# akuendig/cuda-matrix-inversion

Hardware: AMD Instinct MI355X
Metric: matrix inversions/s (higher is better)
Workload: dtype f64; 1 GPU; gj64: 100000 x 64x64 fp64 Gauss-Jordan, SPD inputs (natural-order pivots verified inside the MFMA sweep; a rejected matrix is redone with partial pivoting), BASELINE configs[2]; n=64, total_batch=100000, batch_per_gpu=100000, algorithm=gj, kernel=matinv_gj_tile_f64<4, true, true>, input=SPD: R + R^T + n I

## Files before the change

### cuda-matrix-inversion_amd/csrc/tile_gj_kernels.hip

```cpp
#include "tile_impl.hpp"

namespace matinv {

template hipError_t launch_gj_tile<double>(int, BatchRef<const double>, BatchRef<double>, size_t, int *, hipStream_t);

}
```

### cuda-matrix-inversion_amd/csrc/tile_impl.hpp

```cpp
#pragma once
#include <stdio.h>
#include <stdlib.h>
#include <string.h>
#include <atomic>

#include "tile_common.hpp"
#include "tile_screen.hpp"

#ifndef MATINV_TILE_GATED_PANEL
#define MATINV_TILE_GATED_PANEL 1
#endif

#ifndef MATINV_TILE_SYM_SWEEP
#define MATINV_TILE_SYM_SWEEP 1
#endif

namespace matinv {


#define MATINV_PREP_ROW(MOV, b, a) MOV " %" #b ", %" #a "\n\t" MOV " %" #a ", 0\n\t"
#define MATINV_PREP_ZERO(MOV, a) MOV " %" #a ", 0\n\t"
#define MATINV_PREP_TAIL(MOV, save, eye) MOV " %0, %" #eye "\n\ts_nop 1\n\ts_mov_b64 exec, %" #save
#define MATINV_PREP_SAVE(save, mask) "s_and_saveexec_b64 %" #save ", %" #mask "\n\t"
template <int NT, class T>
__device__ __forceinline__ void prep_operands(typename TileGeo<T>::vec4 (&acc)[NT][NT], T (&bop)[NT], int kb, T eye)
{
    static_assert(NT >= 1 && NT <= 4, "prep_operands: one asm text per tile count");
    const int tK = kb >> 2, rK = kb & 3;
    const unsigned long long pmask = sizeof(T) == 8 ? 0x000F000F000F000FULL << (4 * rK) : 0x1111111111111111ULL << rK;
    unsigned long long save;
    auto J = [&](int i) { return (tK + i) % NT; };
    auto R = [&](int i) { return (rK + i) & 3; };
#define ROW(i) acc[tK][J(i)][rK]
#define COL(i, r) acc[J(i)][tK][R(r)]
    if constexpr (sizeof(T) == 8) {
#define MV "v_mov_b64_e32"
        if constexpr (NT == 1)
            asm volatile(MATINV_PREP_ROW(MV, 0, 1) MATINV_PREP_SAVE(5, 6)
                         MATINV_PREP_ZERO(MV, 2) MATINV_PREP_ZERO(MV, 3) MATINV_PREP_ZERO(MV, 4) MATINV_PREP_TAIL(MV, 5, 7)
                         : "=&v"(bop[J(0)]), "+v"(ROW(0)), "+v"(COL(0, 1)), "+v"(COL(0, 2)), "+v"(COL(0, 3)), "=&s"(save)
                         : "s"(pmask), "v"(eye) : "scc");
        else if constexpr (NT == 2)
            asm volatile(MATINV_PREP_ROW(MV, 0, 2) MATINV_PREP_ROW(MV, 1, 3) MATINV_PREP_SAVE(11, 12)
                         MATINV_PREP_ZERO(MV, 4) MATINV_PREP_ZERO(MV, 5) MATINV_PREP_ZERO(MV, 6)
                         MATINV_PREP_ZERO(MV, 7) MATINV_PREP_ZERO(MV, 8) MATINV_PREP_ZERO(MV, 9) MATINV_PREP_ZERO(MV, 10)
                         MATINV_PREP_TAIL(MV, 11, 13)
                         : "=&v"(bop[J(0)]), "=&v"(bop[J(1)]), "+v"(ROW(0)), "+v"(ROW(1)),
                           "+v"(COL(0, 1)), "+v"(COL(0, 2)), "+v"(COL(0, 3)),
                           "+v"(COL(1, 0)), "+v"(COL(1, 1)), "+v"(COL(1, 2)), "+v"(COL(1, 3)), "=&s"(save)
                         : "s"(pmask), "v"(eye) : "scc");
        else if constexpr (NT == 3)
            asm volatile(MATINV_PREP_ROW(MV, 0, 3) MATINV_PREP_ROW(MV, 1, 4) MATINV_PREP_ROW(MV, 2, 5) MATINV_PREP_SAVE(17, 18)
                         MATINV_PREP_ZERO(MV, 6) MATINV_PREP_ZERO(MV, 7) MATINV_PREP_ZERO(MV, 8)
                         MATINV_PREP_ZERO(MV, 9) MATINV_PREP_ZERO(MV, 10) MATINV_PREP_ZERO(MV, 11) MATINV_PREP_ZERO(MV, 12)
                         MATINV_PREP_ZERO(MV, 13) MATINV_PREP_ZERO(MV, 14) MATINV_PREP_ZERO(MV, 15) MATINV_PREP_ZERO(MV, 16)
                         MATINV_PREP_TAIL(MV, 17, 19)
                         : "=&v"(bop[J(0)]), "=&v"(bop[J(1)]), "=&v"(bop[J(2)]), "+v"(ROW(0)), "+v"(ROW(1)), "+v"(ROW(2)),
                           "+v"(COL(0, 1)), "+v"(COL(0, 2)), "+v"(COL(0, 3)),
                           "+v"(COL(1, 0)), "+v"(COL(1, 1)), "+v"(COL(1, 2)), "+v"(COL(1, 3)),
                           "+v"(COL(2, 0)), "+v"(COL(2, 1)), "+v"(COL(2, 2)), "+v"(COL(2, 3)), "=&s"(save)
                         : "s"(pmask), "v"(eye) : "scc");
        else
            asm volatile(MATINV_PREP_ROW(MV, 0, 4) MATINV_PREP_ROW(MV, 1, 5) MATINV_PREP_ROW(MV, 2, 6) MATINV_PREP_ROW(MV, 3, 7)
                         MATINV_PREP_SAVE(23, 24)
                         MATINV_PREP_ZERO(MV, 8) MATINV_PREP_ZERO(MV, 9) MATINV_PREP_ZERO(MV, 10)
                         MATINV_PREP_ZERO(MV, 11) MATINV_PREP_ZERO(MV, 12) MATINV_PREP_ZERO(MV, 13) MATINV_PREP_ZERO(MV, 14)
                         MATINV_PREP_ZERO(MV, 15) MATINV_PREP_ZERO(MV, 16) MATINV_PREP_ZERO(MV, 17) MATINV_PREP_ZERO(MV, 18)
                         MATINV_PREP_ZERO(MV, 19) MATINV_PREP_ZERO(MV, 20) MATINV_PREP_ZERO(MV, 21) MATINV_PREP_ZERO(MV, 22)
                         MATINV_PREP_TAIL(MV, 23, 25)
                         : "=&v"(bop[J(0)]), "=&v"(bop[J(1)]), "=&v"(bop[J(2)]), "=&v"(bop[J(3)]),
                           "+v"(ROW(0)), "+v"(ROW(1)), "+v"(ROW(2)), "+v"(ROW(3)),
                           "+v"(COL(0, 1)), "+v"(COL(0, 2)), "+v"(COL(0, 3)),
                           "+v"(COL(1, 0)), "+v"(COL(1, 1)), "+v"(COL(1, 2)), "+v"(COL(1, 3)),
                           "+v"(COL(2, 0)), "+v"(COL(2, 1)), "+v"(COL(2, 2)), "+v"(COL(2, 3)),
                           "+v"(COL(3, 0)), "+v"(COL(3, 1)), "+v"(COL(3, 2)), "+v"(COL(3, 3)), "=&s"(save)
                         : "s"(pmask), "v"(eye) : "scc");
#undef MV
    } else {
#define MV "v_mov_b32_e32"
        if constexpr (NT == 1)
            asm volatile(MATINV_PREP_ROW(MV, 0, 1) MATINV_PREP_SAVE(5, 6)
                         MATINV_PREP_ZERO(MV, 2) MATINV_PREP_ZERO(MV, 3) MATINV_PREP_ZERO(MV, 4) MATINV_PREP_TAIL(MV, 5, 7)
                         : "=&v"(bop[J(0)]), "+v"(ROW(0)), "+v"(COL(0, 1)), "+v"(COL(0, 2)), "+v"(COL(0, 3)), "=&s"(save)
                         : "s"(pmask), "v"(eye) : "scc");
        else if constexpr (NT == 2)
            asm volatile(MATINV_PREP_ROW(MV, 0, 2) MATINV_PREP_ROW(MV, 1, 3) MATINV_PREP_SAVE(11, 12)
                         MATINV_PREP_ZERO(MV, 4) MATINV_PREP_ZERO(MV, 5) MATINV_PREP_ZERO(MV, 6)
                         MATINV_PREP_ZERO(MV, 7) MATINV_PREP_ZERO(MV, 8) MATINV_PREP_ZERO(MV, 9) MATINV_PREP_ZERO(MV, 10)
                         MATINV_PREP_TAIL(MV, 11, 13)
                         : "=&v"(bop[J(0)]), "=&v"(bop[J(1)]), "+v"(ROW(0)), "+v"(ROW(1)),
                           "+v"(COL(0, 1)), "+v"(COL(0, 2)), "+v"(COL(0, 3)),
                           "+v"(COL(1, 0)), "+v"(COL(1, 1)), "+v"(COL(1, 2)), "+v"(COL(1, 3)), "=&s"(save)
                         : "s"(pmask), "v"(eye) : "scc");
        else if constexpr (NT == 3)
            asm volatile(MATINV_PREP_ROW(MV, 0, 3) MATINV_PREP_ROW(MV, 1, 4) MATINV_PREP_ROW(MV, 2, 5) MATINV_PREP_SAVE(17, 18)
                         MATINV_PREP_ZERO(MV, 6) MATINV_PREP_ZERO(MV, 7) MATINV_PREP_ZERO(MV, 8)
                         MATINV_PREP_ZERO(MV, 9) MATINV_PREP_ZERO(MV, 10) MATINV_PREP_ZERO(MV, 11) MATINV_PREP_ZERO(MV, 12)
                         MATINV_PREP_ZERO(MV, 13) MATINV_PREP_ZERO(MV, 14) MATINV_PREP_ZERO(MV, 15) MATINV_PREP_ZERO(MV, 16)
                         MATINV_PREP_TAIL(MV, 17, 19)
                         : "=&v"(bop[J(0)]), "=&v"(bop[J(1)]), "=&v"(bop[J(2)]), "+v"(ROW(0)), "+v"(ROW(1)), "+v"(ROW(2)),
                           "+v"(COL(0, 1)), "+v"(COL(0, 2)), "+v"(COL(0, 3)),
                           "+v"(COL(1, 0)), "+v"(COL(1, 1)), "+v"(COL(1, 2)), "+v"(COL(1, 3)),
                           "+v"(COL(2, 0)), "+v"(COL(2, 1)), "+v"(COL(2, 2)), "+v"(COL(2, 3)), "=&s"(save)
                         : "s"(pmask), "v"(eye) : "scc");
        else
            asm volatile(MATINV_PREP_ROW(MV, 0, 4) MATINV_PREP_ROW(MV, 1, 5) MATINV_PREP_ROW(MV, 2, 6) MATINV_PREP_ROW(MV, 3, 7)
                         MATINV_PREP_SAVE(23, 24)
                         MATINV_PREP_ZERO(MV, 8) MATINV_PREP_ZERO(MV, 9) MATINV_PREP_ZERO(MV, 10)
                         MATINV_PREP_ZERO(MV, 11) MATINV_PREP_ZERO(MV, 12) MATINV_PREP_ZERO(MV, 13) MATINV_PREP_ZERO(MV, 14)
                         MATINV_PREP_ZERO(MV, 15) MATINV_PREP_ZERO(MV, 16) MATINV_PREP_ZERO(MV, 17) MATINV_PREP_ZERO(MV, 18)
                         MATINV_PREP_ZERO(MV, 19) MATINV_PREP_ZERO(MV, 20) MATINV_PREP_ZERO(MV, 21) MATINV_PREP_ZERO(MV, 22)
                         MATINV_PREP_TAIL(MV, 23, 25)
                         : "=&v"(bop[J(0)]), "=&v"(bop[J(1)]), "=&v"(bop[J(2)]), "=&v"(bop[J(3)]),
                           "+v"(ROW(0)), "+v"(ROW(1)), "+v"(ROW(2)), "+v"(ROW(3)),
                           "+v"(COL(0, 1)), "+v"(COL(0, 2)), "+v"(COL(0, 3)),
                           "+v"(COL(1, 0)), "+v"(COL(1, 1)), "+v"(COL(1, 2)), "+v"(COL(1, 3)),
                           "+v"(COL(2, 0)), "+v"(COL(2, 1)), "+v"(COL(2, 2)), "+v"(COL(2, 3)),
                           "+v"(COL(3, 0)), "+v"(COL(3, 1)), "+v"(COL(3, 2)), "+v"(COL(3, 3)), "=&s"(save)
                         : "s"(pmask), "v"(eye) : "scc");
#undef MV
    }
#undef ROW
#undef COL
}
#undef MATINV_PREP_ROW
#undef MATINV_PREP_ZERO
#undef MATINV_PREP_TAIL
#undef MATINV_PREP_SAVE


__device__ __forceinline__ void note_differs(unsigned long long &asym, double a, double b)
{
    asm volatile("v_cmp_ne_u64_e64 vcc, %1, %2\n\ts_or_b64 %0, %0, vcc" : "+s"(asym) : "v"(a), "v"(b) : "vcc");
}

template <int NT>
__device__ __forceinline__ unsigned long long tile_asymmetry(double *tbuf, const v4d (&acc)[NT][NT], int q, int c)
{
    typedef TileGeo<double> G;
    unsigned long long asym = 0;
#pragma unroll
    for (int ti = 0; ti < NT; ++ti)
#pragma unroll
        for (int tj = 0; tj <= ti; ++tj) {
            if (asym != 0) continue;
            wave_lds_sync();
#pragma unroll
            for (int r = 0; r < 4; ++r) tbuf[G::trow(r, q) * TILE_TSTRIDE + c] = acc[ti][tj][r];
            wave_lds_sync();
#pragma unroll
            for (int r = 0; r < 4; ++r) note_differs(asym, tbuf[c * TILE_TSTRIDE + G::trow(r, q)], acc[tj][ti][r]);
        }
    return asym;
}

__device__ __forceinline__ void pin_tiles(v4d (&acc)[4][4])
{
    asm volatile("" : "+v"(acc[0][0]), "+v"(acc[0][1]), "+v"(acc[0][2]), "+v"(acc[0][3]), "+v"(acc[1][0]), "+v"(acc[1][1]),
                      "+v"(acc[1][2]), "+v"(acc[1][3]), "+v"(acc[2][0]), "+v"(acc[2][1]), "+v"(acc[2][2]), "+v"(acc[2][3]),
                      "+v"(acc[3][0]), "+v"(acc[3][1]), "+v"(acc[3][2]), "+v"(acc[3][3]));
}

template <int NT, bool GATED, class T>
__device__ __forceinline__ void sym_tile_sweep(typename TileGeo<T>::vec4 (&acc)[NT][NT], T *panel, int q, int c, unsigned long long &bad)
{
    typedef TileGeo<T> G;
    typedef PanelSolve<NT, false, T, GATED, true> PS;
    constexpr int NKB = 4 * NT;
    T aop[NT], bop[NT];
    spd_panel_to_lds<NT, T>(panel, acc, 0, q, c);
    wave_lds_sync();
    {
        PS ps0;
#pragma unroll
        for (int s = 0; s < PS::NSTAGE; ++s) ps0.stage(s, panel, 0, q, c, aop, bop, bad);
    }
#pragma unroll
    for (int kb = 0; kb < NKB; ++kb) {
        spd_prep_operands<NT, T>(acc, bop, kb, q, c);
        if (kb + 1 < NKB) {
            const int tn = (kb + 1) >> 2;
#pragma unroll
            for (int ti = tn; ti < NT; ++ti) acc[ti][tn] = G::mfma(aop[ti], bop[tn], acc[ti][tn]);
#pragma unroll
            for (int tj = 0; tj < tn; ++tj) acc[tn][tj] = G::mfma(aop[tn], bop[tj], acc[tn][tj]);
            constexpr int NB = NT * (NT + 1) / 2 - NT;
            constexpr int NS = PS::NSTAGE;
            T aop_next[NT], bop_next[NT];
            PS ps;
            int count = 0, ev = 0;
            auto run_events = [&](bool flush) {
#pragma unroll
                for (int e = 0; e < NS + 1; ++e) {
                    const int lead = NB < 2 ? NB : 2;
                    const int thr = (e == 0) ? lead : lead + ((NB - lead) * e) / NS;
                    if (e == ev && (flush || thr <= count)) {
                        __builtin_amdgcn_sched_barrier(0);
                        if (e == 0) {
                            wave_lds_sync();
                            spd_panel_to_lds<NT, T>(panel, acc, kb + 1, q, c);
                            wave_lds_sync();
                        } else {
                            ps.stage(e - 1, panel, kb + 1, q, c, aop_next, bop_next, bad);
                        }
                        __builtin_amdgcn_sched_barrier(0);
                        ++ev;
                    }
                }
            };
            run_events(false);
#pragma unroll
            for (int ti = 0; ti < NT; ++ti)
#pragma unroll
                for (int tj = 0; tj <= ti; ++tj) {
                    if (ti == tn || tj == tn) continue;
                    acc[ti][tj] = G::mfma(aop[ti], bop[tj], acc[ti][tj]);
                    ++count;
                    run_events(false);
                }
            run_events(true);
#pragma unroll
            for (int ti = 0; ti < NT; ++ti) { aop[ti] = aop_next[ti]; bop[ti] = bop_next[ti]; }
        } else {
#pragma unroll
            for (int ti = 0; ti < NT; ++ti)
#pragma unroll
                for (int tj = 0; tj <= ti; ++tj) acc[ti][tj] = G::mfma(aop[ti], bop[tj], acc[ti][tj]);
        }
    }
}

template <int NT>
__device__ __forceinline__ void sym_tile_finish(double *tbuf, v4d (&acc)[NT][NT], int q, int c)
{
    typedef TileGeo<double> G;
#pragma unroll
    for (int ti = 0; ti < NT; ++ti)
#pragma unroll
        for (int tj = 0; tj <= ti; ++tj) {
            acc[ti][tj] = -acc[ti][tj];
            wave_lds_sync();
#pragma unroll
            for (int r = 0; r < 4; ++r) tbuf[G::trow(r, q) * TILE_TSTRIDE + c] = acc[ti][tj][r];
            wave_lds_sync();
#pragma unroll
            for (int r = 0; r < 4; ++r) {
                const double t = tbuf[c * TILE_TSTRIDE + G::trow(r, q)];
                acc[tj][ti][r] = (ti != tj || G::trow(r, q) < c) ? t : acc[tj][ti][r];
            }
        }
}

template <class T, int NT, bool FULL, bool LOOKAHEAD, bool EARLY = false>
__device__ __forceinline__ void gj_tile_body(BatchRef<const T> Ain, BatchRef<T> Xout, int *info, int n_rt, unsigned batch,
                                             int *work_count, int *work_list, T *panel, const int *in_count, const int *in_list)
{
    typedef TileGeo<T> G;
    typedef typename G::vec4 vec4;
    typedef typename G::vec2 vec2;
    constexpr int N = 16 * NT;
    constexpr int NKB = 4 * NT;
    constexpr bool PAIRED = FULL && (NT % 2 == 0);
    constexpr bool GATED = MATINV_TILE_GATED_PANEL && sizeof(T) == 8 && NT == 4 && FULL && LOOKAHEAD && !EARLY;
    constexpr bool SYM = MATINV_TILE_SYM_SWEEP && sizeof(T) == 8 && NT == 4 && FULL && LOOKAHEAD;
    const int l = threadIdx.x;

    const unsigned todo = in_count ? (unsigned)*in_count : batch;
    for (unsigned item = blockIdx.x; item < todo; item += gridDim.x) {
        const unsigned mat = in_list ? (unsigned)in_list[item] : item;
        const T *A = Ain.at_uniform(mat);
        T *X = Xout.at_uniform(mat);
        int n = FULL ? N : n_rt;
        if (!FULL) asm volatile("" : "+s"(n));
        int q = l >> 4, c = l & 15;
        const unsigned lane_off = (unsigned)(G::trow(0, l >> 4) * n + (l & 15));
        asm volatile("" : "+v"(q), "+v"(c));
        const T eye = G::piv(c) == q ? (T)1 : (T)0;
        vec4 acc[NT][NT];
        if (PAIRED) {
            const unsigned lane_off2 = (unsigned)(2 * G::trow(0, l >> 4) * N + 2 * (l & 15));
#pragma unroll
            for (int ti = 0; ti < NT; ++ti)
#pragma unroll
                for (int u = 0; u < NT / 2; ++u)
#pragma unroll
                    for (int r = 0; r < 4; ++r) {
                        const unsigned uoff = (unsigned)((32 * (ti >> 1) + 2 * G::trow(r, 0) + (ti & 1)) * N + 32 * u);
                        const vec2 v = __builtin_nontemporal_load(reinterpret_cast<const vec2 *>(A + uoff + lane_off2));
                        acc[ti][2 * u][r] = v[0];
                        acc[ti][2 * u + 1][r] = v[1];
                    }
        } else {
#pragma unroll
            for (int ti = 0; ti < NT; ++ti)
#pragma unroll
                for (int tj = 0; tj < NT; ++tj)
#pragma unroll
                    for (int r = 0; r < 4; ++r) {
                        const int row = 16 * ti + G::trow(r, q), col = 16 * tj + c;
                        const unsigned uoff = (unsigned)((16 * ti + G::trow(r, 0)) * n + 16 * tj);
                        const bool edge = !FULL && (ti == NT - 1 || tj == NT - 1);
                        acc[ti][tj][r] = (!edge || (row < n && col < n)) ? A[uoff + lane_off] : ((row == col) ? (T)1 : (T)0);
                    }
        }
        unsigned long long bad = 0;
        T aop[NT], bop[NT];

        bool sym = false;
#ifndef MATINV_TILE_LDST_ONLY
        if constexpr (SYM) {
            pin_tiles(acc);
            sym = tile_asymmetry<NT>(panel, acc, q, c) == 0;
        }
#endif

#ifdef MATINV_TILE_LDST_ONLY
        if (false) {
#else
        if (SYM && sym) {
        } else if (LOOKAHEAD) {
#endif
            panel_to_lds<NT, T>(panel, acc, 0, q, c);
            wave_lds_sync();
            panel_solve<NT, GATED>(panel, 0, q, c, aop, bad);
#pragma unroll
            for (int kb = 0; kb < NKB; ++kb) {
                if (!FULL && kb > 4 * (NT - 1) && kb - 4 * (NT - 1) >= G::real_blocks(n - 16 * (NT - 1))) continue;
                prep_operands<NT, T>(acc, bop, kb, eye);
                if (kb + 1 < NKB) {
                    const int tn = (kb + 1) >> 2;
#pragma unroll
                    for (int ti = 0; ti < NT; ++ti)
                        acc[ti][tn] = G::mfma(aop[ti], bop[tn], acc[ti][tn]);
                    constexpr int NB = NT * (NT - 1);
                    int pend = 0;
                    auto issue_b = [&](int count) {
#pragma unroll
                        for (int z = 0; z < count; ++z) {
                            if (pend < NB) {
                                const int tjx = pend / NT, ti = pend % NT;
                                const int tj = tjx + (tjx >= tn ? 1 : 0);
                                acc[ti][tj] = G::mfma(aop[ti], bop[tj], acc[ti][tj]);
                                ++pend;
                            }
                        }
                        __builtin_amdgcn_sched_barrier(0);
                    };
                    __builtin_amdgcn_sched_barrier(0);
                    issue_b(2);
                    wave_lds_sync();
                    panel_to_lds<NT, T>(panel, acc, kb + 1, q, c);
                    wave_lds_sync();
                    __builtin_amdgcn_sched_barrier(0);
                    T aop_next[NT];
                    PanelSolve<NT, false, T, GATED> ps;
                    constexpr int NS = PanelSolve<NT, false, T, GATED>::NSTAGE;
#pragma unroll
                    for (int s = 0; s < NS; ++s) {
                        issue_b(((NB - 2) * (s + 1)) / NS - ((NB - 2) * s) / NS);
                        ps.stage(s, panel, kb + 1, q, c, aop_next, bad);
                        __builtin_amdgcn_sched_barrier(0);
                    }
                    issue_b(NB);
#pragma unroll
                    for (int ti = 0; ti < NT; ++ti) aop[ti] = aop_next[ti];
                    if (EARLY && NT > 1 && kb == 3 && bad != 0) break;
                } else {
#pragma unroll
                    for (int ti = 0; ti < NT; ++ti)
#pragma unroll
                        for (int tj = 0; tj < NT; ++tj)
                            acc[ti][tj] = G::mfma(aop[ti], bop[tj], acc[ti][tj]);
                }
            }
        } else {
#ifdef MATINV_TILE_LDST_ONLY
            (void)aop, (void)bop;
#else
#pragma unroll
            for (int kb = 0; kb < NKB; ++kb) {
                if (!FULL && kb > 4 * (NT - 1) && kb - 4 * (NT - 1) >= G::real_blocks(n - 16 * (NT - 1))) continue;
                panel_to_lds<NT, T>(panel, acc, kb, q, c);
                wave_lds_sync();
                panel_solve<NT>(panel, kb, q, c, aop, bad);
                wave_lds_sync();
                prep_operands<NT, T>(acc, bop, kb, eye);
#pragma unroll
                for (int ti = 0; ti < NT; ++ti)
#pragma unroll
                    for (int tj = 0; tj < NT; ++tj)
                        acc[ti][tj] = G::mfma(aop[ti], bop[tj], acc[ti][tj]);
            }
#endif
        }

#define MATINV_GJ_TILE_LEAVE                                                                                                \
        if (bad == 0) {                                                                                                     \
            if (PAIRED) {                                                                                                   \
                const unsigned lane_off2 = (unsigned)(2 * G::trow(0, l >> 4) * N + 2 * (l & 15));                           \
_Pragma("unroll")                                                                                                           \
                for (int ti = 0; ti < NT; ++ti)                                                                             \
_Pragma("unroll")                                                                                                           \
                    for (int u = 0; u < NT / 2; ++u)                                                                        \
_Pragma("unroll")                                                                                                           \
                        for (int r = 0; r < 4; ++r) {                                                                       \
                            const unsigned uoff = (unsigned)((32 * (ti >> 1) + 2 * G::trow(r, 0) + (ti & 1)) * N + 32 * u); \
                            vec2 v;                                                                                         \
                            v[0] = acc[ti][2 * u][r];                                                                       \
                            v[1] = acc[ti][2 * u + 1][r];                                                                   \
                            __builtin_nontemporal_store(v, reinterpret_cast<vec2 *>(X + uoff + lane_off2));                 \
                        }                                                                                                   \
            } else {                                                                                                        \
_Pragma("unroll")                                                                                                           \
                for (int ti = 0; ti < NT; ++ti)                                                                             \
_Pragma("unroll")                                                                                                           \
                    for (int tj = 0; tj < NT; ++tj)                                                                         \
_Pragma("unroll")                                                                                                           \
                        for (int r = 0; r < 4; ++r) {                                                                       \
                            const int row = 16 * ti + G::trow(r, q), col = 16 * tj + c;                                     \
                            const unsigned uoff = (unsigned)((16 * ti + G::trow(r, 0)) * n + 16 * tj);                      \
                            const bool edge = !FULL && (ti == NT - 1 || tj == NT - 1);                                      \
                            if (!edge || (row < n && col < n)) X[uoff + lane_off] = acc[ti][tj][r];                         \
                        }                                                                                                   \
            }                                                                                                               \
            if (info && l == 0) info[mat] = 0;                                                                              \
        } else if (l == 0) {                                                                                                \
            const int slot = atomicAdd(work_count, 1);                                                                      \
            work_list[slot] = (int)mat;                                                                                     \
        }
        if constexpr (SYM) {
            auto leave = [&]() {
                MATINV_GJ_TILE_LEAVE
            };
            if (!sym) {
                leave();
            } else {
                int qs = q, cs = c;
                asm volatile("" : "+v"(qs), "+v"(cs));
                wave_lds_sync();
                sym_tile_sweep<NT, MATINV_TILE_GATED_PANEL != 0, T>(acc, panel, qs, cs, bad);
                wave_lds_sync();
                if (bad == 0) sym_tile_finish<NT>(panel, acc, qs, cs);
                leave();
            }
        } else {
            MATINV_GJ_TILE_LEAVE
        }
#undef MATINV_GJ_TILE_LEAVE
        if (LOOKAHEAD) wave_lds_sync();
    }
}


template <int NT, bool FULL, bool LOOKAHEAD, bool EARLY = false>
__global__ __launch_bounds__(64, 2) void matinv_gj_tile_f64(BatchRef<const double> Ain,
                                                                                 BatchRef<double> Xout, int *info,
                                                                                 int n_rt, unsigned batch,
                                                                                 int *work_count, int *work_list, const int *in_count,
                                                                                 const int *in_list)
{
    constexpr bool SYM = MATINV_TILE_SYM_SWEEP && NT == 4 && FULL && LOOKAHEAD;
    __shared__ __attribute__((aligned(16))) double panel[SYM && 16 * NT * 4 < 16 * TILE_TSTRIDE ? 16 * TILE_TSTRIDE : 16 * NT * 4];
    gj_tile_body<double, NT, FULL, LOOKAHEAD, EARLY>(Ain, Xout, info, n_rt, batch, work_count, work_list, panel, in_count, in_list);
}

template <int NT, bool FULL, bool LOOKAHEAD, bool EARLY = false>
__global__ __launch_bounds__(64, FULL ? 4 : 3) void matinv_gj_tile_f32(BatchRef<const float> Ain, BatchRef<float> Xout, int *info,
                                                           int n_rt, unsigned batch, int *work_count, int *work_list, const int *in_count,
                                                           const int *in_list)
{
    __shared__ __attribute__((aligned(16))) float panel[16 * NT * 4];
    gj_tile_body<float, NT, FULL, LOOKAHEAD, EARLY>(Ain, Xout, info, n_rt, batch, work_count, work_list, panel, in_count, in_list);
}

template <class T>
struct SpdGp {
    const T *a, *c, *d, *e;
    T *out;
};

template <class T, int NT, bool FULL, bool GP = false>
__device__ __forceinline__ void spd_tile_body(BatchRef<const T> Ain, BatchRef<T> Xout, int *info, int n_rt, unsigned batch,
                                              int *work_count, int *work_list, T *panel, SpdGp<T> gp = SpdGp<T>())
{
    typedef TileGeo<T> G;
    typedef typename G::vec4 vec4;
    constexpr int N = 16 * NT;
    constexpr int NKB = 4 * NT;
    constexpr int TSTRIDE = TILE_TSTRIDE;
    const int l = threadIdx.x;

    for (unsigned mat = blockIdx.x; mat < batch; mat += gridDim.x) {
        const T *A = Ain.at_uniform(mat);
        T *X = Xout.at_uniform(mat);
        int n = FULL ? N : n_rt;
        if (!FULL) asm volatile("" : "+s"(n));
        int q = l >> 4, c = l & 15;
        const unsigned lane_off = (unsigned)((l >> 4) * n + (l & 15));
        asm volatile("" : "+v"(q), "+v"(c));

        vec4 acc[NT][NT];
#pragma unroll
        for (int ti = 0; ti < NT; ++ti)
#pragma unroll
            for (int tj = 0; tj < NT; ++tj) {
                if (tj > ti) continue;
#pragma unroll
                for (int r = 0; r < 4; ++r) {
                    const int row = 16 * ti + G::trow(r, q), col = 16 * tj + c;
                    T v;
                    if (ti == tj) {
                        const int hi = row > col ? row : col, lo = row > col ? col : row;
                        v = (FULL || ti < NT - 1 || (row < n && col < n)) ? A[(unsigned)(lo * n + hi)] : ((row == col) ? (T)1 : (T)0);
                        if (GP && row == col && (FULL || ti < NT - 1 || row < n)) v += gp.c[(size_t)mat * n + row];
                    } else {
                        v = (FULL || ti < NT - 1 || (row < n && col < n)) ? A[(unsigned)(col * n + row)] : (T)0;
                    }
                    acc[ti][tj][r] = v;
                }
            }
        (void)lane_off;
        unsigned long long bad = 0;
        T aop[NT], bop[NT];

        spd_panel_to_lds<NT, T>(panel, acc, 0, q, c);
        wave_lds_sync();
        {
            PanelSolve<NT, true, T> ps0;
#pragma unroll
            for (int s = 0; s < PanelSolve<NT, true, T>::NSTAGE; ++s) ps0.stage(s, panel, 0, q, c, aop, bop, bad);
        }
#pragma unroll
        for (int kb = 0; kb < NKB; ++kb) {
            const int tK = kb >> 2;
            if (!FULL && kb > 4 * (NT - 1) && kb - 4 * (NT - 1) >= G::real_blocks(n - 16 * (NT - 1))) continue;
            spd_prep_operands<NT, T>(acc, bop, kb, q, c);
            if (kb + 1 < NKB) {
                const int tn = (kb + 1) >> 2;
#pragma unroll
                for (int ti = 0; ti < NT; ++ti) {
                    if (ti < tn) continue;
                    acc[ti][tn] = G::mfma(aop[ti], bop[tn], acc[ti][tn]);
                }
#pragma unroll
                for (int tj = 0; tj < NT; ++tj) {
                    if (tj >= tn) continue;
                    acc[tn][tj] = G::mfma(aop[tn], bop[tj], acc[tn][tj]);
                }
                constexpr int NB = NT * (NT + 1) / 2 - NT;
                constexpr int NS = PanelSolve<NT, true, T>::NSTAGE;
                T aop_next[NT], bop_next[NT];
                PanelSolve<NT, true, T> ps;
                int count = 0, ev = 0;
                auto run_events = [&](bool flush) {
#pragma unroll
                    for (int e = 0; e < NS + 1; ++e) {
                        const int lead = NB < 2 ? NB : 2;
                        const int thr = (e == 0) ? lead : lead + ((NB - lead) * e) / NS;
                        if (e == ev && (flush || thr <= count)) {
                            __builtin_amdgcn_sched_barrier(0);
                            if (e == 0) {
                                wave_lds_sync();
                                spd_panel_to_lds<NT, T>(panel, acc, kb + 1, q, c);
                                wave_lds_sync();
                            } else {
                                ps.stage(e - 1, panel, kb + 1, q, c, aop_next, bop_next, bad);
                            }
                            __builtin_amdgcn_sched_barrier(0);
                            ++ev;
                        }
                    }
                };
                run_events(false);
#pragma unroll
                for (int ti = 0; ti < NT; ++ti)
#pragma unroll
                    for (int tj = 0; tj < NT; ++tj) {
                        if (tj > ti || ti == tn || tj == tn) continue;
                        acc[ti][tj] = G::mfma(aop[ti], bop[tj], acc[ti][tj]);
                        ++count;
                        run_events(false);
                    }
                run_events(true);
#pragma unroll
                for (int ti = 0; ti < NT; ++ti) { aop[ti] = aop_next[ti]; bop[ti] = bop_next[ti]; }
            } else {
#pragma unroll
                for (int ti = 0; ti < NT; ++ti)
#pragma unroll
                    for (int tj = 0; tj < NT; ++tj) {
                        if (tj > ti) continue;
                        acc[ti][tj] = G::mfma(aop[ti], bop[tj], acc[ti][tj]);
                    }
            }
            (void)tK;
        }

        if (GP && bad == 0) {
            const T *va = gp.a + (size_t)mat * n;
            const T *vd = gp.d ? gp.d + (size_t)mat * n : va;
            wave_lds_sync();
            T *const sa = panel, *const sd = panel + N;
#pragma unroll
            for (int k = 0; k < (N + 63) / 64; ++k) {
                const int i = l + 64 * k;
                if (i < N) {
                    sa[i] = (FULL || i < n) ? va[i] : (T)0;
                    sd[i] = (FULL || i < n) ? vd[i] : (T)0;
                }
            }
            wave_lds_sync();
            T s = 0;
#pragma unroll
            for (int tj = 0; tj < NT; ++tj) {
                const T ac = sa[16 * tj + c], dc = sd[16 * tj + c];
#pragma unroll
                for (int ti = tj; ti < NT; ++ti)
#pragma unroll
                    for (int r = 0; r < 4; ++r) {
                        const int row = 16 * ti + G::trow(r, q);
                        const T ar = sa[row], dr = sd[row];
                        const T wgt = (ti == tj) ? ar * dc : fma_t(ar, dc, dr * ac);
                        s = fma_t(acc[ti][tj][r], wgt, s);
                    }
            }
#pragma unroll
            for (int off = 32; off >= 1; off >>= 1) s += __shfl_xor(s, off);
            if (l == 0) {
                gp.out[mat] = gp.d ? -s : gp.e[mat] + s;
                if (info) info[mat] = 0;
            }
        } else if (bad == 0) {
#pragma unroll
            for (int ti = 0; ti < NT; ++ti)
#pragma unroll
                for (int tj = 0; tj < NT; ++tj) {
                    if (tj > ti) continue;
#pragma unroll
                    for (int r = 0; r < 4; ++r) {
                        const int row = 16 * ti + G::trow(r, q), col = 16 * tj + c;
                        if (FULL || ti < NT - 1 || (row < n && col < n)) X[(unsigned)(row * n + col)] = -acc[ti][tj][r];
                    }
                    if (tj < ti) {
                        wave_lds_sync();
#pragma unroll
                        for (int r = 0; r < 4; ++r) panel[G::trow(r, q) * TSTRIDE + c] = -acc[ti][tj][r];
                        wave_lds_sync();
#pragma unroll
                        for (int r = 0; r < 4; ++r) {
                            const int row = 16 * tj + G::trow(r, q), col = 16 * ti + c;
                            const T v = panel[c * TSTRIDE + G::trow(r, q)];
                            if (FULL || ti < NT - 1 || (row < n && col < n)) X[(unsigned)(row * n + col)] = v;
                        }
                    }
                }
            if (info && l == 0) info[mat] = 0;
        } else if (l == 0) {
            const int slot = atomicAdd(work_count, 1);
            work_list[slot] = (int)mat;
        }
        wave_lds_sync();
    }
}


template <int NT, bool FULL>
__global__ __launch_bounds__(64, NT >= 7 ? 1 : (NT >= 5 ? 2 : (NT >= 4 ? 3 : 4))) void matinv_spd_tile_f64(BatchRef<const double> Ain, BatchRef<double> Xout,
                                                                          int *info, int n_rt, unsigned batch,
                                                                          int *work_count, int *work_list)
{
    __shared__ __attribute__((aligned(16))) double panel[(16 * NT * 4 > 16 * 17) ? 16 * NT * 4 : 16 * 17];
    spd_tile_body<double, NT, FULL>(Ain, Xout, info, n_rt, batch, work_count, work_list, panel);
}

template <int NT, bool FULL>
#ifndef MATINV_SPD_WIDE_OCC
#define MATINV_SPD_WIDE_OCC 2
#endif
__global__ __launch_bounds__(64, NT >= 9 ? MATINV_SPD_WIDE_OCC : (NT >= 7 ? 2 : (NT >= 5 ? 3 : 4))) void matinv_spd_tile_f32(BatchRef<const float> Ain, BatchRef<float> Xout, int *info,
                                                            int n_rt, unsigned batch, int *work_count, int *work_list)
{
    __shared__ __attribute__((aligned(16))) float panel[(16 * NT * 4 > 16 * 17) ? 16 * NT * 4 : 16 * 17];
    spd_tile_body<float, NT, FULL>(Ain, Xout, info, n_rt, batch, work_count, work_list, panel);
}

template <int NT>
__global__ __launch_bounds__(64, NT >= 7 ? 1 : 2) void matinv_gp_spd_tile_f64(const double *As, const double *Bs, const double *Cs, const double *Ds,
                                                               const double *Es, double *out, int *info, int n_rt, unsigned batch,
                                                               int *work_count, int *work_list)
{
    __shared__ __attribute__((aligned(16))) double panel[(16 * NT * 4 > 16 * 17) ? 16 * NT * 4 : 16 * 17];
    BatchRef<const double> A{Bs, (size_t)n_rt * n_rt, nullptr};
    BatchRef<double> X{nullptr, 0, nullptr};
    spd_tile_body<double, NT, false, true>(A, X, info, n_rt, batch, work_count, work_list, panel, SpdGp<double>{As, Cs, Ds, Es, out});
}
template <int NT>
__global__ __launch_bounds__(64, NT >= 9 ? MATINV_SPD_WIDE_OCC : 2) void matinv_gp_spd_tile_f32(const float *As, const float *Bs, const float *Cs, const float *Ds,
                                                               const float *Es, float *out, int *info, int n_rt, unsigned batch,
                                                               int *work_count, int *work_list)
{
    __shared__ __attribute__((aligned(16))) float panel[(16 * NT * 4 > 16 * 17) ? 16 * NT * 4 : 16 * 17];
    BatchRef<const float> A{Bs, (size_t)n_rt * n_rt, nullptr};
    BatchRef<float> X{nullptr, 0, nullptr};
    spd_tile_body<float, NT, false, true>(A, X, info, n_rt, batch, work_count, work_list, panel, SpdGp<float>{As, Cs, Ds, Es, out});
}


bool tile_policy_use_screen(bool f64, int nt);
template <class T>
hipError_t launch_gj_tile_natural(int n, BatchRef<const T> A, BatchRef<T> X, size_t batch, int *info, hipStream_t stream)
{
    constexpr bool F64 = sizeof(T) == 8;
    const TileShape s = tile_shape(n);
    const bool rowlane2 = rowlane2_supports(n);
    const bool screen = !rowlane2 && tile_policy_use_screen(F64, s.nt);
    return with_scratch_ints((screen ? 3 : 2) * batch + 4, 4, stream, [&](int *ws) {
        int *const rej_count = ws, *const sing_count = ws + 1, *const acc_count = ws + 2;
        int *const rej_list = ws + 4, *const sing_list = ws + 4 + batch, *const acc_list = ws + 4 + 2 * batch;
        hipError_t e;
        if (rowlane2) {
            e = enqueue_gj_rowlane2<T>(n, A, X, batch, info, stream, rej_count, rej_list);
        } else {
            const unsigned grid = tile_grid(batch, F64 ? 8u : 16u), b = (unsigned)batch;
            const unsigned sgrid = tile_grid(batch, 16u, 1u);
            with_tile<1, 4>(s, [&](auto NT, auto FULL) {
                constexpr bool EARLY = NT >= 3;
                if constexpr (F64) {
                    if (!screen) {
                        hipLaunchKernelGGL((matinv_gj_tile_f64<NT, FULL, true>), dim3(grid), dim3(64), 0, stream, A, X, info, n, b, rej_count,
                                           rej_list, nullptr, nullptr);
                        return;
                    }
                    hipLaunchKernelGGL((matinv_gj_tile_screen_f64<NT, FULL>), dim3(sgrid), dim3(64), 0, stream, A, n, b, rej_count, rej_list,
                                       acc_count, acc_list);
                    hipLaunchKernelGGL((matinv_gj_tile_f64<NT, FULL, true, EARLY>), dim3(grid), dim3(64), 0, stream, A, X, info, n, b, rej_count,
                                       rej_list, acc_count, acc_list);
                } else {
                    if (!screen) {
                        hipLaunchKernelGGL((matinv_gj_tile_f32<NT, FULL, true>), dim3(grid), dim3(64), 0, stream, A, X, info, n, b, rej_count,
                                           rej_list, nullptr, nullptr);
                        return;
                    }
                    hipLaunchKernelGGL((matinv_gj_tile_screen_f32<NT, FULL>), dim3(sgrid), dim3(64), 0, stream, A, n, b, rej_count, rej_list,
                                       acc_count, acc_list);
                    hipLaunchKernelGGL((matinv_gj_tile_f32<NT, FULL, true, EARLY>), dim3(grid), dim3(64), 0, stream, A, X, info, n, b, rej_count,
                                       rej_list, acc_count, acc_list);
                }
            });
            e = hipGetLastError();
        }
        if (e == hipSuccess)
            e = launch_gj_tilep_worklist<T>(n, A, X, batch, rej_count, rej_list, sing_count, sing_list, info, stream,
                                            tile_policy_record(F64, s.nt, batch), screen);
        return e;
    });
}

template <class T>
hipError_t launch_gj_tile(int n, BatchRef<const T> A, BatchRef<T> X, size_t batch, int *info, hipStream_t stream)
{
    if (!tile_family_supports<T>(n)) return hipErrorInvalidValue;
    if (batch == 0) return hipSuccess;
    if (n > 64) return launch_gj_tile4<T>(n, A, X, batch, info, stream);
    if (tile_policy_use_pivot(sizeof(T) == 8, tile_shape(n).nt)) return launch_gj_tilep<T>(n, A, X, batch, info, stream);
    return launch_gj_tile_natural<T>(n, A, X, batch, info, stream);
}

constexpr TileShape spd_tile_shape(bool f64, int n) { return {(n + 15) / 16, n % 16 == 0 && (f64 || n < 128)}; }

hipError_t enqueue_spd_tile_big_f32(int n, BatchRef<const float> A, BatchRef<float> X, unsigned grid, unsigned b, int *info, int *ws,
                                    hipStream_t stream);
template <class T>
hipError_t launch_gp_spd_tile(int n, const T *As, const T *Bs, const T *Cs, const T *Ds, const T *Es, T *out, size_t batch, int *info,
                              hipStream_t stream)
{
    if (!gp_spd_tile_supports(sizeof(T) == 8, n)) return hipErrorInvalidValue;
    if (batch == 0) return hipSuccess;
    return with_scratch_ints(batch + 1, 1, stream, [&](int *ws) {
        const unsigned grid = tile_grid(batch, 8u), b = (unsigned)batch;
        hipError_t e = hipSuccess;
        if constexpr (sizeof(T) == 8) {
            if (n <= 96) hipLaunchKernelGGL((matinv_gp_spd_tile_f64<6>), dim3(grid), dim3(64), 0, stream, As, Bs, Cs, Ds, Es, out, info, n, b, ws, ws + 1);
            else e = enqueue_gp_spd_tile_wide_f64(n, As, Bs, Cs, Ds, Es, out, grid, b, info, ws, stream);
        } else {
            if (n <= 112) hipLaunchKernelGGL((matinv_gp_spd_tile_f32<7>), dim3(grid), dim3(64), 0, stream, As, Bs, Cs, Ds, Es, out, info, n, b, ws, ws + 1);
            else if (n <= 128) hipLaunchKernelGGL((matinv_gp_spd_tile_f32<8>), dim3(grid), dim3(64), 0, stream, As, Bs, Cs, Ds, Es, out, info, n, b, ws, ws + 1);
            else e = enqueue_gp_spd_tile_wide_f32(n, As, Bs, Cs, Ds, Es, out, grid, b, info, ws, stream);
        }
        if (e == hipSuccess) e = hipGetLastError();
        if (e == hipSuccess) e = launch_gp_lds_worklist<T>(n, As, Bs, Cs, Ds, Es, out, ws, ws + 1, info, stream);
        return e;
    });
}

}
```

Baseline: 76.85 million inversions/s.

## Batch symmetric tile transposes through LDS and prefetch panel rows in sym sweep

The symmetry check and the final mirror step now transpose up to three tiles per LDS round in four rounds, where before each of the ten tiles took its own pair of wave barriers. This cuts the number of LDS syncs and lets the reads overlap. A new SymPanelSolve subclass prefetches panel row weights into registers during stage 0, so the later stages skip their LDS reads. The cost is more LDS (three transpose slots) and more registers, which could reduce occupancy. Optional cycle-counter phase stamps are also added behind a macro.

```diff
diff --git a/cuda-matrix-inversion_amd/csrc/tile_gj_kernels.hip b/cuda-matrix-inversion_amd/csrc/tile_gj_kernels.hip
--- a/cuda-matrix-inversion_amd/csrc/tile_gj_kernels.hip
+++ b/cuda-matrix-inversion_amd/csrc/tile_gj_kernels.hip
@@ -5,3 +5,13 @@
 template hipError_t launch_gj_tile<double>(int, BatchRef<const double>, BatchRef<double>, size_t, int *, hipStream_t);
 
 }
+
+#ifdef MATINV_TILE_PHASE_STAMPS
+extern "C" int matinv_phase_stamps_read(unsigned long long *dst, size_t mats)
+{
+    if (mats > matinv::PHASE_STAMP_MATS) return -1;
+    if (hipDeviceSynchronize() != hipSuccess) return -3;
+    return hipMemcpyFromSymbol(dst, HIP_SYMBOL(matinv::g_phase_stamps), mats * matinv::PHASE_STAMP_POINTS * sizeof(unsigned long long), 0,
+                               hipMemcpyDeviceToHost) == hipSuccess ? 0 : -3;
+}
+#endif
diff --git a/cuda-matrix-inversion_amd/csrc/tile_impl.hpp b/cuda-matrix-inversion_amd/csrc/tile_impl.hpp
--- a/cuda-matrix-inversion_amd/csrc/tile_impl.hpp
+++ b/cuda-matrix-inversion_amd/csrc/tile_impl.hpp
@@ -3,6 +3,7 @@
 #include <stdlib.h>
 #include <string.h>
 #include <atomic>
+#include <type_traits>
 
 #include "tile_common.hpp"
 #include "tile_screen.hpp"
@@ -15,7 +16,28 @@
 #define MATINV_TILE_SYM_SWEEP 1
 #endif
 
+#ifndef MATINV_TILE_SYM_LDS_BATCH
+#define MATINV_TILE_SYM_LDS_BATCH 1
+#endif
+
+#ifndef MATINV_TILE_SYM_ROW_PREFETCH
+#define MATINV_TILE_SYM_ROW_PREFETCH MATINV_TILE_SYM_LDS_BATCH
+#endif
+
 namespace matinv {
+
+#ifdef MATINV_TILE_PHASE_STAMPS
+constexpr unsigned PHASE_STAMP_MATS = 1u << 17;
+constexpr int PHASE_STAMP_POINTS = 7;
+static __device__ unsigned long long g_phase_stamps[PHASE_STAMP_MATS * PHASE_STAMP_POINTS];
+#define MATINV_STAMP(k)                                                                                                    \
+    if constexpr (SYM) {                                                                                                   \
+        const unsigned long long t_ = __builtin_readcyclecounter();                                                        \
+        if (l == 0 && mat < PHASE_STAMP_MATS) g_phase_stamps[mat * PHASE_STAMP_POINTS + (k)] = t_;                         \
+    }
+#else
+#define MATINV_STAMP(k)
+#endif
 
 
 #define MATINV_PREP_ROW(MOV, b, a) MOV " %" #b ", %" #a "\n\t" MOV " %" #a ", 0\n\t"
@@ -134,11 +156,44 @@
     asm volatile("v_cmp_ne_u64_e64 vcc, %1, %2\n\ts_or_b64 %0, %0, vcc" : "+s"(asym) : "v"(a), "v"(b) : "vcc");
 }
 
+constexpr int SYM_TSLOTS = MATINV_TILE_SYM_LDS_BATCH ? 3 : 1;
+constexpr int SYM_TSLOT = 16 * TILE_TSTRIDE;
+constexpr int SYM_NROUND = 4;
+constexpr int sym_order_ti(int k) { const int t[10] = {1, 0, 1, 2, 2, 2, 3, 3, 3, 3}; return t[k]; }
+constexpr int sym_order_tj(int k) { const int t[10] = {0, 0, 1, 0, 1, 2, 0, 1, 2, 3}; return t[k]; }
+constexpr int sym_round_begin(int g) { return g == 0 ? 0 : 1 + 3 * (g - 1); }
+
 template <int NT>
 __device__ __forceinline__ unsigned long long tile_asymmetry(double *tbuf, const v4d (&acc)[NT][NT], int q, int c)
 {
     typedef TileGeo<double> G;
     unsigned long long asym = 0;
+    if constexpr (MATINV_TILE_SYM_LDS_BATCH != 0) {
+        static_assert(NT == 4, "the round table is written for the ten lower tiles of 4 x 4");
+#pragma unroll
+        for (int g = 0; g < SYM_NROUND; ++g) {
+            if (asym != 0) continue;
+            const int k0 = sym_round_begin(g), k1 = sym_round_begin(g + 1);
+            double t[SYM_TSLOTS][4];
+            wave_lds_sync();
+#pragma unroll
+            for (int k = k0; k < k1; ++k)
+#pragma unroll
+                for (int r = 0; r < 4; ++r)
+                    tbuf[(k - k0) * SYM_TSLOT + G::trow(r, q) * TILE_TSTRIDE + c] = acc[sym_order_ti(k)][sym_order_tj(k)][r];
+            wave_lds_sync();
+#pragma unroll
+            for (int k = k0; k < k1; ++k)
+#pragma unroll
+                for (int r = 0; r < 4; ++r) t[k - k0][r] = tbuf[(k - k0) * SYM_TSLOT + c * TILE_TSTRIDE + G::trow(r, q)];
+            __builtin_amdgcn_sched_barrier(0);
+#pragma unroll
+            for (int k = k0; k < k1; ++k)
+#pragma unroll
+                for (int r = 0; r < 4; ++r) note_differs(asym, t[k - k0][r], acc[sym_order_tj(k)][sym_order_ti(k)][r]);
+        }
+        return asym;
+    }
 #pragma unroll
     for (int ti = 0; ti < NT; ++ti)
 #pragma unroll
@@ -162,18 +217,69 @@
 }
 
 template <int NT, bool GATED, class T>
+struct SymPanelSolve : PanelSolve<NT, false, T, GATED, true> {
+    typedef PanelSolve<NT, false, T, GATED, true> Base;
+    typedef TileGeo<T> G;
+    T pw[NT][4], pb[NT];
+
+    __device__ __forceinline__ void prefetch_rows(const T *panel, int q, int c, int t0, int t1)
+    {
+#pragma unroll
+        for (int ti = t0; ti < t1; ++ti) {
+            const T *w = &panel[(16 * ti + c) * 4];
+#pragma unroll
+            for (int j = 0; j < 4; ++j) pw[ti][j] = w[j];
+            pb[ti] = w[q];
+        }
+    }
+    __device__ __forceinline__ void stage(int s, const T *panel, int kb, int q, int c, T (&aop)[NT], T (&bsym)[NT],
+                                          unsigned long long &bad)
+    {
+        if (s < 6) {
+            Base::stage(s, panel, kb, q, c, aop, bsym, bad);
+            return;
+        }
+        const int tK = kb >> 2, rK = kb & 3;
+        const bool panel_lane = G::blk(c) == rK;
+        const int ti = s - 6;
+        const T w0 = pw[ti][0], w1 = pw[ti][1], w2 = pw[ti][2], w3 = pw[ti][3];
+        T v = fma_t(-w3, this->x3, fma_t(-w2, this->x2, fma_t(-w1, this->x1, -w0 * this->x0)));
+        if (ti == tK) {
+            const int m = G::piv(c);
+            const T x01 = (m & 1) ? this->x1 : this->x0, x23 = (m & 1) ? this->x3 : this->x2;
+            const T xm = (m & 2) ? x23 : x01;
+            note_fail_except(bad, v, __ballot(panel_lane));
+            v = panel_lane ? xm : v;
+        } else {
+            note_fail(bad, v);
+        }
+        aop[ti] = v;
+        bsym[ti] = pb[ti];
+    }
+};
+
+template <int NT, bool GATED, bool ROWPF, class T>
 __device__ __forceinline__ void sym_tile_sweep(typename TileGeo<T>::vec4 (&acc)[NT][NT], T *panel, int q, int c, unsigned long long &bad)
 {
     typedef TileGeo<T> G;
-    typedef PanelSolve<NT, false, T, GATED, true> PS;
+    typedef typename std::conditional<ROWPF, SymPanelSolve<NT, GATED, T>, PanelSolve<NT, false, T, GATED, true>>::type PS;
     constexpr int NKB = 4 * NT;
     T aop[NT], bop[NT];
+    auto stage_pf = [&](PS &p, int s, int kb, T (&a)[NT], T (&b)[NT]) {
+        if constexpr (ROWPF) {
+            if (s == 0) p.prefetch_rows(panel, q, c, 0, NT / 2);
+            p.stage(s, panel, kb, q, c, a, b, bad);
+            if (s == 0) p.prefetch_rows(panel, q, c, NT / 2, NT);
+        } else {
+            p.stage(s, panel, kb, q, c, a, b, bad);
+        }
+    };
     spd_panel_to_lds<NT, T>(panel, acc, 0, q, c);
     wave_lds_sync();
     {
         PS ps0;
 #pragma unroll
-        for (int s = 0; s < PS::NSTAGE; ++s) ps0.stage(s, panel, 0, q, c, aop, bop, bad);
+        for (int s = 0; s < PS::NSTAGE; ++s) stage_pf(ps0, s, 0, aop, bop);
     }
 #pragma unroll
     for (int kb = 0; kb < NKB; ++kb) {
@@ -201,7 +307,7 @@
                             spd_panel_to_lds<NT, T>(panel, acc, kb + 1, q, c);
                             wave_lds_sync();
                         } else {
-                            ps.stage(e - 1, panel, kb + 1, q, c, aop_next, bop_next, bad);
+                            stage_pf(ps, e - 1, kb + 1, aop_next, bop_next);
                         }
                         __builtin_amdgcn_sched_barrier(0);
                         ++ev;
@@ -234,6 +340,34 @@
 __device__ __forceinline__ void sym_tile_finish(double *tbuf, v4d (&acc)[NT][NT], int q, int c)
 {
     typedef TileGeo<double> G;
+    if constexpr (MATINV_TILE_SYM_LDS_BATCH != 0) {
+        static_assert(NT == 4, "the round table is written for the ten lower tiles of 4 x 4");
+#pragma unroll
+        for (int g = 0; g < SYM_NROUND; ++g) {
+            const int k0 = sym_round_begin(g), k1 = sym_round_begin(g + 1);
+            double t[SYM_TSLOTS][4];
+            wave_lds_sync();
+#pragma unroll
+            for (int k = k0; k < k1; ++k) {
+                const int ti = sym_order_ti(k), tj = sym_order_tj(k);
+                acc[ti][tj] = -acc[ti][tj];
+#pragma unroll
+                for (int r = 0; r < 4; ++r) tbuf[(k - k0) * SYM_TSLOT + G::trow(r, q) * TILE_TSTRIDE + c] = acc[ti][tj][r];
+            }
+            wave_lds_sync();
+#pragma unroll
+            for (int k = k0; k < k1; ++k)
+#pragma unroll
+                for (int r = 0; r < 4; ++r) t[k - k0][r] = tbuf[(k - k0) * SYM_TSLOT + c * TILE_TSTRIDE + G::trow(r, q)];
+#pragma unroll
+            for (int k = k0; k < k1; ++k) {
+                const int ti = sym_order_ti(k), tj = sym_order_tj(k);
+#pragma unroll
+                for (int r = 0; r < 4; ++r) acc[tj][ti][r] = (ti != tj || G::trow(r, q) < c) ? t[k - k0][r] : acc[tj][ti][r];
+            }
+        }
+        return;
+    }
 #pragma unroll
     for (int ti = 0; ti < NT; ++ti)
 #pragma unroll
@@ -272,6 +406,7 @@
         T *X = Xout.at_uniform(mat);
         int n = FULL ? N : n_rt;
         if (!FULL) asm volatile("" : "+s"(n));
+        MATINV_STAMP(0)
         int q = l >> 4, c = l & 15;
         const unsigned lane_off = (unsigned)(G::trow(0, l >> 4) * n + (l & 15));
         asm volatile("" : "+v"(q), "+v"(c));
@@ -305,6 +440,11 @@
         }
         unsigned long long bad = 0;
         T aop[NT], bop[NT];
+        MATINV_STAMP(1)
+#ifdef MATINV_TILE_PHASE_STAMPS
+        if constexpr (SYM) asm volatile("s_waitcnt vmcnt(0)" ::: "memory");
+#endif
+        MATINV_STAMP(2)
 
         bool sym = false;
 #ifndef MATINV_TILE_LDST_ONLY
@@ -313,6 +453,7 @@
             sym = tile_asymmetry<NT>(panel, acc, q, c) == 0;
         }
 #endif
+        MATINV_STAMP(3)
 
 #ifdef MATINV_TILE_LDST_ONLY
         if (false) {
@@ -438,15 +579,19 @@
                 int qs = q, cs = c;
                 asm volatile("" : "+v"(qs), "+v"(cs));
                 wave_lds_sync();
-                sym_tile_sweep<NT, MATINV_TILE_GATED_PANEL != 0, T>(acc, panel, qs, cs, bad);
+                sym_tile_sweep<NT, MATINV_TILE_GATED_PANEL != 0, MATINV_TILE_SYM_ROW_PREFETCH != 0, T>(acc, panel, qs, cs, bad);
                 wave_lds_sync();
+                MATINV_STAMP(4)
                 if (bad == 0) sym_tile_finish<NT>(panel, acc, qs, cs);
+                MATINV_STAMP(5)
                 leave();
             }
+            MATINV_STAMP(6)
         } else {
             MATINV_GJ_TILE_LEAVE
         }
 #undef MATINV_GJ_TILE_LEAVE
+#undef MATINV_STAMP
         if (LOOKAHEAD) wave_lds_sync();
     }
 }
@@ -460,7 +605,7 @@
                                                                                  const int *in_list)
 {
     constexpr bool SYM = MATINV_TILE_SYM_SWEEP && NT == 4 && FULL && LOOKAHEAD;
-    __shared__ __attribute__((aligned(16))) double panel[SYM && 16 * NT * 4 < 16 * TILE_TSTRIDE ? 16 * TILE_TSTRIDE : 16 * NT * 4];
+    __shared__ __attribute__((aligned(16))) double panel[SYM && 16 * NT * 4 < SYM_TSLOTS * SYM_TSLOT ? SYM_TSLOTS * SYM_TSLOT : 16 * NT * 4];
     gj_tile_body<double, NT, FULL, LOOKAHEAD, EARLY>(Ain, Xout, info, n_rt, batch, work_count, work_list, panel, in_count, in_list);
 }
 
```

Result: no change. 77.09 million inversions/s, median of 6 (+0.3%).
